# linusmossberg/monte-carlo-ray-tracer

Measured on NVIDIA H100. Metric: Mray/s (primary+shadow+bounce), higher is better.
Workload: dtype f64

## Files before the change

### include/mcrt_abi.h

```cpp
#ifndef MCRT_ABI_H
#define MCRT_ABI_H

#include <stddef.h>
#include <stdint.h>

#ifdef __cplusplus
extern "C" {
#endif

#define MCRT_ABI_VERSION 1

typedef enum mcrt_status {
    MCRT_OK = 0,
    MCRT_ERR_INVALID = -1,
    MCRT_ERR_CUDA = -2,
    MCRT_ERR_NO_SCENE = -3,
    MCRT_ERR_UNSUPPORTED = -4,
    MCRT_ERR_NO_PHOTONS = -5
} mcrt_status;

enum { MCRT_PRIM_TRIANGLE = 0, MCRT_PRIM_SPHERE = 1, MCRT_PRIM_QUADRIC = 2 };

enum { MCRT_INTEGRATOR_PATH = 0, MCRT_INTEGRATOR_PHOTON = 1 };

// ... 305 lines not shown
#define MCRT_DENOISE_DEFAULT_SIGMA_DEPTH 0.1
#define MCRT_DENOISE_DEFAULT_SIGMA_ALBEDO 0.1

int mcrt_denoise_dev(mcrt_ctx* ctx, const double* a_rgb_dev, const double* a_weight_dev,
                     const double* b_rgb_dev, const double* b_weight_dev, const uint32_t* tile_samples,
                     uint32_t tile, const double* features_dev, uint32_t width, uint32_t height,
                     const mcrt_denoise_params* params, double* out_rgb_dev, double* frame_error);

int mcrt_denoise_planes_dev(mcrt_ctx* ctx, const double* a_rgb_dev, const double* b_rgb_dev,
                            const double* a_planes_dev, const double* b_planes_dev, uint32_t n_planes,
                            const uint32_t* tile_samples, uint32_t tile, const double* features_dev,
                            uint32_t width, uint32_t height, const mcrt_denoise_params* params,
                            double* a_out_planes_dev, double* b_out_planes_dev,
                            double* out_rgb_dev, double* frame_error);

int mcrt_frame_alloc(mcrt_ctx* ctx, uint64_t bytes, void** dev_ptr, unsigned char ipc_handle[64]);
int mcrt_frame_open(mcrt_ctx* ctx, const unsigned char ipc_handle[64], void** dev_ptr);
int mcrt_frame_close(mcrt_ctx* ctx, void* peer_ptr);
int mcrt_frame_free(mcrt_ctx* ctx, void* dev_ptr);

int mcrt_bvh4_host(const mcrt_scene_desc* scene, uint32_t max_leaf, void** handle, const void** nodes128, uint32_t* n_nodes);
void mcrt_bvh4_host_free(void* handle);

int mcrt_fp64_peak(mcrt_ctx* ctx, double* dfma_per_second);

int mcrt_trace_closest(mcrt_ctx* ctx, const mcrt_ray* rays, size_t n, int precision,
                       mcrt_hit* hits, mcrt_stats* stats);

int mcrt_sample_rays(mcrt_ctx* ctx, const mcrt_ray* rays, const uint32_t* pixel,
                     const uint32_t* sample, size_t n, uint32_t global_seed,
                     int integrator_kind, int precision, double* out_rgb, mcrt_stats* stats);

int mcrt_sampler_stream(mcrt_ctx* ctx, const uint32_t* pixel, const uint32_t* sample, size_t n,
                        uint32_t n_shuffles, uint32_t global_seed, uint32_t* out_u32x7);

int mcrt_knn_search(mcrt_ctx* ctx, int which, const double* points_xyz, size_t n,
                    uint32_t* out_index, double* out_dist2, uint32_t* out_count,
                    mcrt_stats* stats);

int mcrt_set_option(mcrt_ctx* ctx, const char* key, double value);

#ifdef __cplusplus
}
#endif
#endif
```

### monte-carlo-ray-tracer_b200/__init__.py

```python
import ctypes as C
import math
import os
import struct

import numpy as np

HERE = os.path.dirname(os.path.abspath(__file__))
LIB_PATH = os.environ.get("MCRT_LIB", os.path.join(HERE, "libmcrt_b200.so"))

INTEGRATOR_PATH, INTEGRATOR_PHOTON = 0, 1
PRECISION_F64, PRECISION_F32 = 0, 1
PRIM_TRIANGLE, PRIM_SPHERE, PRIM_QUADRIC = 0, 1, 2
NO_PRIM = 0xFFFFFFFF

ABI_SYMBOLS = [
    "mcrt_abi_version", "mcrt_init", "mcrt_destroy", "mcrt_last_error", "mcrt_scene_upload",
    "mcrt_photon_upload", "mcrt_photon_emit", "mcrt_photon_download", "mcrt_octree_build",
    "mcrt_octree_free", "mcrt_render_rows", "mcrt_render_rows_dev", "mcrt_render_rows_strided_dev",
    "mcrt_trace_closest",
    "mcrt_sample_rays", "mcrt_sampler_stream", "mcrt_knn_search", "mcrt_set_option", "mcrt_set_film",
    "mcrt_obj_load", "mcrt_obj_free", "mcrt_obj_vertex_normals",
    "mcrt_bvh_build", "mcrt_bvh_free", "mcrt_image_tonemap", "mcrt_image_tonemap_dev",
    "mcrt_render_rows_strided_peers", "mcrt_frame_alloc", "mcrt_frame_open", "mcrt_frame_close", "mcrt_frame_free",
    "mcrt_render_film_sums_strided_dev", "mcrt_film_resolve_dev",
    "mcrt_bvh4_host", "mcrt_bvh4_host_free",
    "mcrt_fp64_peak", "mcrt_photon_emit_total", "mcrt_photon_emit_range", "mcrt_photon_build_dev",
    "mcrt_render_accumulate_dev", "mcrt_progressive_resolve_dev",
    "mcrt_render_accumulate_tiles_dev", "mcrt_progressive_resolve_tiles_dev",
    "mcrt_render_features_dev", "mcrt_denoise_dev", "mcrt_render_features_chain_dev",
    "mcrt_photon_emit_pass", "mcrt_photon_gather_radius", "mcrt_photon_gather_search",
    "mcrt_set_light_groups", "mcrt_render_accumulate_groups_dev", "mcrt_light_groups_combine_dev",
    "mcrt_render_accumulate_aovs_dev", "mcrt_photon_download_lights", "mcrt_render_accumulate_photon_components_dev",
    "mcrt_set_light_path_expressions", "mcrt_render_accumulate_lpe_dev", "mcrt_lpe_compile_host",
    "mcrt_lpe_compile_photon_host", "mcrt_photon_download_lpe_states", "mcrt_denoise_planes_dev",
]

AOV_NAMES = ("background", "emission", "diffuse_direct", "diffuse_indirect", "reflection_direct", "reflection_indirect",
             "transmission_direct", "transmission_indirect")

PHOTON_COMPONENT_NAMES = ("emission", "direct", "caustic", "global")

LPE_SYM_RD, LPE_SYM_RS, LPE_SYM_RG, LPE_SYM_TS, LPE_SYM_TG, LPE_SYM_B, LPE_SYM_L, LPE_SYM_LABEL0 = range(8)
LPE_DEAD, LPE_MAX_STATES, LPE_MAX_SYMBOLS, LPE_MAX_EXPRESSIONS = 255, 255, 71, 32
AOV_LPES = ("CB", "CL", "C<RD>[LB]", "C<RD>.+[LB]", "C[<RS><RG>][LB]", "C[<RS><RG>].+[LB]", "C<T.>[LB]", "C<T.>.+[LB]")


def PM_COMPONENT_LPES(direct_visualization):
    n = "[<RD><RG><TG>]"
# ... 161 lines not shown
        L.mcrt_photon_download.argtypes = [C.c_void_p, C.c_int, C.POINTER(PhotonMapDesc)]
        L.mcrt_photon_download_lights.argtypes = [C.c_void_p, C.c_int, C.c_void_p, C.c_uint64]
        L.mcrt_photon_download_lpe_states.argtypes = [C.c_void_p, C.c_int, C.c_void_p, C.c_uint64]
        L.mcrt_octree_build.argtypes = [C.c_void_p, C.c_void_p, C.c_uint64, C.c_uint32, C.c_void_p, C.POINTER(C.c_void_p),
                                        C.POINTER(PhotonMapDesc), C.POINTER(C.c_double)]
        L.mcrt_octree_free.argtypes = [C.c_void_p]
        L.mcrt_octree_free.restype = None
        render_args = [C.c_void_p, C.POINTER(CameraRec), C.c_uint32, C.c_uint32, C.c_uint32, C.c_uint32,
                       C.c_int, C.c_int, C.c_void_p, C.POINTER(Stats)]
        L.mcrt_render_rows.argtypes = render_args
        L.mcrt_render_rows_dev.argtypes = render_args
        L.mcrt_render_rows_strided_dev.argtypes = [C.c_void_p, C.POINTER(CameraRec), C.c_uint32, C.c_uint32, C.c_uint32,
                                                   C.c_uint32, C.c_uint32, C.c_int, C.c_int, C.c_void_p, C.POINTER(Stats)]
        L.mcrt_render_rows_strided_peers.argtypes = [C.c_void_p, C.POINTER(CameraRec), C.c_uint32, C.c_uint32, C.c_uint32, C.c_uint32,
                                                     C.c_uint32, C.c_int, C.c_int, C.c_void_p, C.c_uint32, C.c_int, C.POINTER(Stats)]
        L.mcrt_frame_alloc.argtypes = [C.c_void_p, C.c_uint64, C.POINTER(C.c_void_p), C.c_void_p]
        L.mcrt_frame_open.argtypes = [C.c_void_p, C.c_void_p, C.POINTER(C.c_void_p)]
        L.mcrt_frame_close.argtypes = [C.c_void_p, C.c_void_p]
        L.mcrt_frame_free.argtypes = [C.c_void_p, C.c_void_p]
        L.mcrt_fp64_peak.argtypes = [C.c_void_p, C.POINTER(C.c_double)]
        L.mcrt_bvh4_host.argtypes = [C.POINTER(SceneDesc), C.c_uint32, C.POINTER(C.c_void_p), C.POINTER(C.c_void_p), C.POINTER(C.c_uint32)]
        L.mcrt_bvh4_host_free.argtypes = [C.c_void_p]
        L.mcrt_bvh4_host_free.restype = None
        L.mcrt_render_film_sums_strided_dev.argtypes = [C.c_void_p, C.POINTER(CameraRec), C.c_uint32, C.c_uint32, C.c_uint32, C.c_uint32,
                                                        C.c_uint32, C.c_int, C.c_int, C.c_void_p, C.c_void_p, C.POINTER(Stats)]
        L.mcrt_film_resolve_dev.argtypes = [C.c_void_p, C.c_void_p, C.c_void_p, C.c_uint64, C.c_void_p]
        L.mcrt_render_accumulate_dev.argtypes = [C.c_void_p, C.POINTER(CameraRec), C.c_uint32, C.c_uint32, C.c_uint32, C.c_uint32,
                                                 C.c_uint32, C.c_uint32, C.c_int, C.c_int, C.c_void_p, C.c_void_p, C.POINTER(Stats)]
        L.mcrt_progressive_resolve_dev.argtypes = [C.c_void_p, C.c_void_p, C.c_void_p, C.c_uint64, C.c_void_p, C.c_void_p, C.c_uint64,
                                                   C.c_uint32, C.c_uint32, C.c_uint32, C.c_void_p, C.c_void_p, C.POINTER(C.c_double)]
        L.mcrt_render_accumulate_tiles_dev.argtypes = [C.c_void_p, C.POINTER(CameraRec), C.c_uint32, C.c_uint32, C.c_uint32, C.c_uint32,
                                                       C.c_void_p, C.c_uint32, C.c_uint32, C.c_uint32, C.c_int, C.c_int, C.c_void_p,
                                                       C.c_void_p, C.POINTER(Stats)]
        L.mcrt_progressive_resolve_tiles_dev.argtypes = [C.c_void_p, C.c_void_p, C.c_void_p, C.c_void_p, C.c_void_p, C.c_void_p,
                                                         C.c_uint32, C.c_uint32, C.c_uint32, C.c_void_p, C.c_void_p, C.c_void_p,
                                                         C.POINTER(C.c_double)]
        L.mcrt_set_light_groups.argtypes = [C.c_void_p, C.c_void_p, C.c_uint32, C.c_uint32]
        L.mcrt_render_accumulate_groups_dev.argtypes = [C.c_void_p, C.POINTER(CameraRec), C.c_uint32, C.c_uint32, C.c_uint32, C.c_uint32,
                                                        C.c_void_p, C.c_uint32, C.c_uint32, C.c_uint32, C.c_int, C.c_int, C.c_void_p,
                                                        C.c_uint32, C.POINTER(Stats)]
        L.mcrt_render_accumulate_aovs_dev.argtypes = L.mcrt_render_accumulate_groups_dev.argtypes
        L.mcrt_render_accumulate_photon_components_dev.argtypes = L.mcrt_render_accumulate_groups_dev.argtypes
        L.mcrt_set_light_path_expressions.argtypes = [C.c_void_p, C.c_void_p, C.c_uint32]
        L.mcrt_render_accumulate_lpe_dev.argtypes = L.mcrt_render_accumulate_groups_dev.argtypes
        L.mcrt_lpe_compile_host.argtypes = [C.c_void_p, C.c_uint32, C.c_uint32, C.c_void_p, C.c_void_p, C.c_void_p,
                                            C.POINTER(C.c_uint32), C.POINTER(C.c_uint32), C.c_char_p, C.c_uint32]
# ... 824 lines not shown
                   gpu_ms=ms.value, rounds=int(d.build_rounds), kernel_launches=int(d.kernel_launches))
        lib().mcrt_bvh_free(h)
        return out
    finally:
        lib().mcrt_destroy(ctx)


BVH4_NODE_DTYPE = np.dtype([("lo", "<f4", (3, 4)), ("hi", "<f4", (3, 4)), ("child", "<u4", (4,)), ("pad", "<u4", (4,))])


def bvh4_host(scene, max_leaf=0xFFFFFFFF):
    d = scene.desc()
    h, p, n = C.c_void_p(), C.c_void_p(), C.c_uint32()
    rc = lib().mcrt_bvh4_host(C.byref(d), max_leaf, C.byref(h), C.byref(p), C.byref(n))
    if rc:
        raise McrtError(f"mcrt_bvh4_host failed with {rc}")
    try:
        if n.value == 0:
            return np.zeros(0, BVH4_NODE_DTYPE)
        buf = (C.c_uint8 * (128 * n.value)).from_address(p.value)
        return np.frombuffer(buf, dtype=BVH4_NODE_DTYPE).copy()
    finally:
        lib().mcrt_bvh4_host_free(h)


def _lpe_strings(exprs):
    arr = (C.c_char_p * max(len(exprs), 1))()
    for i, e in enumerate(exprs):
        arr[i] = str(e).encode()
    return arr


def lpe_compile(exprs, n_groups=0):
    exprs = list(exprs)
    arr = _lpe_strings(exprs)
    nxt = np.zeros(LPE_MAX_STATES * LPE_MAX_SYMBOLS, np.uint8)
    acc = np.zeros(256, np.uint32)
    gs = np.zeros(max(int(n_groups), 1), np.uint8)
    ns, nsym = C.c_uint32(), C.c_uint32()
    err = C.create_string_buffer(1024)
    rc = lib().mcrt_lpe_compile_host(C.cast(arr, C.c_void_p) if exprs else None, len(exprs), int(n_groups),
                                     nxt.ctypes.data_as(C.c_void_p), acc.ctypes.data_as(C.c_void_p),
                                     gs.ctypes.data_as(C.c_void_p), C.byref(ns), C.byref(nsym), err, len(err))
    if rc:
        e = McrtError(f"mcrt_lpe_compile_host failed with {rc}: {err.value.decode()}")
        e.code = rc
# ... 596 lines not shown
```

### monte-carlo-ray-tracer_b200/csrc/abi.cu

```cuda
#include <algorithm>
#include <cmath>
#include <cstdio>
#include <cstdlib>
#include <cstring>
#include <string>
#include <vector>

#include "mcrt_abi.h"
#include "launch.h"
#include "bvh_build.h"
#include "image.h"
#include "denoise.h"
#include "lpe.h"

using namespace mcrt;

static const int MCRT_INTERNAL_EMIT = 100;

#define CK(call)                                                                              \
    do {                                                                                      \
        cudaError_t e_ = (call);                                                              \
        if (e_ != cudaSuccess)                                                                \
        {                                                                                     \
            ctx->error = std::string(#call) + ": " + cudaGetErrorString(e_);                  \
            return MCRT_ERR_CUDA;                                                             \
        }                                                                                     \
    } while (0)
// ... 16 lines not shown
    {
        PathBuffer<R> buf[2];
        ShadowRecord<R>* shadow = nullptr;
        V4<R>* hits = nullptr;
        uint32_t capacity = 0;
    };
}

struct mcrt_ctx
{
    int device = 0;
    int sm_count = 132;
    cudaStream_t stream = nullptr;
    std::string error;

    bool has_scene = false;
    std::vector<void*> scene_allocs;
    DeviceScene<double> scene64;
    DeviceScene<float> scene32;
    float scene_scale = 1.0f;
    uint32_t n_bvh4_nodes = 0;
    uint32_t bvh4_max_leaf = 0xFFFFFFFFu;
    int dynamic_fetch = -1;
    PeerFrames peer_out{};
    int exact_traversal = 0;

    WaveBuffers<double> wave64;
    WaveBuffers<float> wave32;
    std::vector<void*> wave_allocs64, wave_allocs32;

    uint32_t* d_sobol_bytes = nullptr;
    Counters* d_counters = nullptr;
    Counters* h_counters = nullptr;
    double* d_film = nullptr;
    size_t film_values = 0;
    bool film_default = true;
    mcrt_film film = {MCRT_FILM_BOX, 0u, 0.5};
    double* d_film_wsum = nullptr;
    size_t film_wsum_values = 0;
    double* d_film_cache = nullptr;
    double* d_host_out = nullptr;
    size_t host_out_values = 0;
    double* d_resolve_scratch = nullptr;
    size_t resolve_scratch_values = 0;
    double* d_denoise_scratch = nullptr;
    size_t denoise_scratch_values = 0;
// ... 392 lines not shown
                {
                    if (!leafRef(kids[c], n.child[c])) return 1;
                }
                else queue.push_back({ kids[c], self, (uint32_t)c });
            }
            out[self] = n;
            return 0;
        };
        std::vector<Item> kids;
        out.emplace_back();
        if (s.node_prim_count[0]) kids.push_back(itemOfNode(0));
        else childrenOf(0, kids);
        bool too_big = emit(kids, 0) != 0;
        for (size_t q = 0; q < queue.size() && !too_big; q++)
        {
            const Pending pn = queue[q];
            const uint32_t self = (uint32_t)out.size();
            out.emplace_back();
            out[pn.parent].child[pn.slot] = self;
            expand(pn.item, kids);
            too_big = emit(kids, self) != 0;
        }
        if (too_big) out.clear();
        return MCRT_OK;
    }

    template <class R>
    int uploadArrays(mcrt_ctx* ctx, const mcrt_scene_desc& s, SceneArrays<R>& a, uint64_t& bytes)
    {
        DeviceScene<R>& d = a.dev;
        int rc;
        if ((rc = devUpload(ctx, ctx->scene_allocs, &d.wide, a.wide, bytes))) return rc;
        if ((rc = devUpload(ctx, ctx->scene_allocs, &d.geom, a.geom, bytes))) return rc;
        if ((rc = devUpload(ctx, ctx->scene_allocs, &d.shade, a.shade, bytes))) return rc;
        if ((rc = devUpload(ctx, ctx->scene_allocs, &d.vnormals, a.vnormals, bytes))) return rc;
        if ((rc = devUpload(ctx, ctx->scene_allocs, &d.quadrics, a.quadrics, bytes))) return rc;
        if ((rc = devUpload(ctx, ctx->scene_allocs, &d.materials, a.materials, bytes))) return rc;
        if ((rc = devUpload(ctx, ctx->scene_allocs, &d.lights, a.lights, bytes))) return rc;
        {
            std::vector<uint32_t> combos;
            std::vector<uint8_t> cls(s.n_prims ? s.n_prims : 1, 1);
            for (uint32_t i = 0; i < s.n_prims; i++)
            {
                const uint32_t combo = (a.materials[a.shade[i].material].flags << 1) | (a.shade[i].vn_index >= 0 ? 1u : 0u);
                size_t k = 0;
                while (k < combos.size() && combos[k] != combo) k++;
// ... 526 lines not shown
            ctx->error = name + ": a reconstruction filter needs weight_sum_dev";
            return MCRT_ERR_INVALID;
        }
        return MCRT_OK;
    }
}

extern "C" int mcrt_photon_upload(mcrt_ctx* ctx, const mcrt_photon_map_desc* caustic_map, const mcrt_photon_map_desc* global_map,
                                  uint32_t k_nearest, uint32_t direct_visualization, uint64_t* h2d_bytes);

extern "C"
{

int mcrt_abi_version(void) { return MCRT_ABI_VERSION; }

int mcrt_init(int device, mcrt_ctx** out_ctx)
{
    if (!out_ctx) return MCRT_ERR_INVALID;
    *out_ctx = nullptr;
    int count = 0;
    if (cudaGetDeviceCount(&count) != cudaSuccess || device < 0 || device >= count) return MCRT_ERR_CUDA;
    mcrt_ctx* ctx = new mcrt_ctx();
    if (const char* e = std::getenv("MCRT_BVH4_MAX_LEAF")) ctx->bvh4_max_leaf = (uint32_t)std::atoi(e);
    ctx->device = device;
    auto fail = [&](int rc) { mcrt_destroy(ctx); return rc; };
    if (cudaSetDevice(device) != cudaSuccess) return fail(MCRT_ERR_CUDA);
    cudaDeviceProp prop;
    if (cudaGetDeviceProperties(&prop, device) != cudaSuccess) return fail(MCRT_ERR_CUDA);
    ctx->sm_count = prop.multiProcessorCount;
    if (cudaStreamCreateWithFlags(&ctx->stream, cudaStreamNonBlocking) != cudaSuccess) return fail(MCRT_ERR_CUDA);
    if (cudaMalloc((void**)&ctx->d_counters, sizeof(Counters)) != cudaSuccess) return fail(MCRT_ERR_CUDA);
    if (cudaMallocHost((void**)&ctx->h_counters, 2 * sizeof(Counters)) != cudaSuccess) return fail(MCRT_ERR_CUDA);
    {
        std::vector<uint32_t> tab(6 * 4 * 256);
        makeSobolByteTable(tab.data());
        if (cudaMalloc((void**)&ctx->d_sobol_bytes, tab.size() * 4) != cudaSuccess) return fail(MCRT_ERR_CUDA);
        if (cudaMemcpy(ctx->d_sobol_bytes, tab.data(), tab.size() * 4, cudaMemcpyHostToDevice) != cudaSuccess) return fail(MCRT_ERR_CUDA);
    }
    if (cudaEventCreate(&ctx->ev_start) != cudaSuccess || cudaEventCreate(&ctx->ev_stop) != cudaSuccess) return fail(MCRT_ERR_CUDA);
    for (int i = 0; i < 2; i++)
        if (cudaEventCreateWithFlags(&ctx->ev_poll[i], cudaEventDisableTiming) != cudaSuccess) return fail(MCRT_ERR_CUDA);
    *out_ctx = ctx;
    return MCRT_OK;
}

void mcrt_destroy(mcrt_ctx* ctx)
// ... 35 lines not shown
    delete ctx;
}

const char* mcrt_last_error(const mcrt_ctx* ctx)
{
    return ctx ? ctx->error.c_str() : "null context";
}

int mcrt_set_option(mcrt_ctx* ctx, const char* key, double value)
{
    if (!ctx || !key) return MCRT_ERR_INVALID;
    std::string k(key);
    if (k == "pool_paths") { if (value < 1024 || value > 268435456.0) return MCRT_ERR_INVALID; ctx->pool_paths = (uint32_t)value; }
    else if (k == "blocks_per_sm") { if (value < 1 || value > 32) return MCRT_ERR_INVALID; ctx->blocks_per_sm = (int)value; }
    else if (k == "ray_eps_scale") { if (value <= 0) return MCRT_ERR_INVALID; ctx->ray_eps_scale = value; }
    else if (k == "poll_interval") { if (value < 1 || value > 1024) return MCRT_ERR_INVALID; ctx->poll_interval = (int)value; }
    else if (k == "stage_timing") { ctx->stage_timing = value != 0.0; }
    else if (k == "sort_rays") { ctx->sort_rays = value != 0.0; }
    else if (k == "sort_shade") { ctx->sort_shade = value != 0.0; }
    else if (k == "sort_shade_class") { ctx->sort_shade_class = value != 0.0; }
    else if (k == "sort_prim_key") { ctx->sort_prim_key = (int)value; }
    else if (k == "exact_traversal") { ctx->exact_traversal = value != 0.0; }
    else if (k == "dynamic_fetch") { ctx->dynamic_fetch = (int)value; }
    else if (k == "bvh4_max_leaf") { if (value < 0 || value > 255) return MCRT_ERR_INVALID; ctx->bvh4_max_leaf = (uint32_t)value; }
    else { ctx->error = "unknown option " + k; return MCRT_ERR_INVALID; }
    return MCRT_OK;
}

int mcrt_scene_upload(mcrt_ctx* ctx, const mcrt_scene_desc* scene, uint64_t* h2d_bytes)
{
    if (!ctx) return MCRT_ERR_INVALID;
    if (!scene || scene->abi_version != MCRT_ABI_VERSION) { ctx->error = "scene description missing or ABI version mismatch"; return MCRT_ERR_INVALID; }
    if (scene->n_prims == 0 || scene->n_materials == 0) { ctx->error = "empty scene"; return MCRT_ERR_INVALID; }
    if (scene->n_prims >= (1u << 24)) { ctx->error = "more than 2^24 primitives"; return MCRT_ERR_UNSUPPORTED; }
    CK(cudaSetDevice(ctx->device));
    const mcrt_scene_desc& s = *scene;

    for (uint32_t i = 0; i < s.n_nodes; i++)
    {
        if (s.node_next_sibling[i] != 0 && (s.node_next_sibling[i] <= i || s.node_next_sibling[i] >= s.n_nodes))
        { ctx->error = "node_next_sibling must point forward"; return MCRT_ERR_INVALID; }
        if ((uint64_t)s.node_first_prim[i] + s.node_prim_count[i] > s.n_prims)
        { ctx->error = "node primitive range out of bounds"; return MCRT_ERR_INVALID; }
        if (s.node_prim_count[i] == 0 && i + 1 >= s.n_nodes)
        { ctx->error = "inner node without children"; return MCRT_ERR_INVALID; }
    }
// ... 34 lines not shown
                double a[3] = { sp[0] - sp[3], sp[1] - sp[3], sp[2] - sp[3] }, b[3] = { sp[0] + sp[3], sp[1] + sp[3], sp[2] + sp[3] };
                add(a); add(b);
            }
            for (uint32_t i = 0; i < s.n_quadrics; i++) { add(s.quadric_bounds + 6 * i); add(s.quadric_bounds + 6 * i + 3); }
        }
        for (int k = 0; k < 3; k++)
        {
            const bool ok = lo[k] <= hi[k] && lo[k] > -1e290 && hi[k] < 1e290;
            ctx->scene_bmin[k] = ok ? lo[k] : -1.0;
            ctx->scene_bmax[k] = ok ? hi[k] : 1.0;
        }
    }

    uint64_t bytes = 0;
    int rc;
    {
        SceneArrays<double> a;
        if ((rc = buildArrays(ctx, s, a))) return rc;
        std::memset(&a.dev, 0, sizeof(a.dev));
        if ((rc = buildWide(ctx, s, a))) return rc;
        if ((rc = uploadArrays(ctx, s, a, bytes))) return rc;
        std::vector<Bvh4Node> bvh4;
        if ((rc = buildBvh4(ctx->bvh4_max_leaf, s, bvh4))) return rc;
        a.dev.bvh4 = nullptr;
        if (!bvh4.empty() && (rc = devUpload(ctx, ctx->scene_allocs, &a.dev.bvh4, bvh4, bytes))) return rc;
        ctx->n_bvh4_nodes = (uint32_t)bvh4.size();
        CK(cudaStreamSynchronize(ctx->stream));
        ctx->scene64 = a.dev;
    }
    {
        SceneArrays<float> a;
        if ((rc = buildArrays(ctx, s, a))) return rc;
        std::memset(&a.dev, 0, sizeof(a.dev));
        if ((rc = buildWide(ctx, s, a))) return rc;
        if ((rc = uploadArrays(ctx, s, a, bytes))) return rc;
        CK(cudaStreamSynchronize(ctx->stream));
        ctx->scene32 = a.dev;
    }
    ctx->prim_interpolates.assign(s.n_prims, 0);
    for (uint32_t i = 0; i < s.n_prims; i++)
        if (s.prim_type[i] == MCRT_PRIM_TRIANGLE && s.tri_vn_index[s.prim_index[i]] >= 0) ctx->prim_interpolates[i] = 1;
    {
        std::vector<uint8_t> lit(s.n_prims, 0);
        for (uint32_t i = 0; i < s.n_lights; i++) lit[s.light_prim[i]] = 1;
        ctx->emissive_unlit = false;
        for (uint32_t i = 0; i < s.n_prims && !ctx->emissive_unlit; i++)
            ctx->emissive_unlit = s.materials[s.prim_material[i]].emissive && !lit[i];
    }
    ctx->has_scene = true;
// ... 1196 lines not shown
{
    if (!ctx) return MCRT_ERR_INVALID;
    if (!rgb_sum_dev || !weight_sum_dev || !out_rgb_dev) { ctx->error = "null buffer"; return MCRT_ERR_INVALID; }
    CK(cudaSetDevice(ctx->device));
    launchResolveFilmWeighted(rgb_sum_dev, weight_sum_dev, out_rgb_dev, n_pixels, ctx->sm_count * ctx->blocks_per_sm, ctx->stream);
    CK(cudaStreamSynchronize(ctx->stream));
    CK(cudaGetLastError());
    return MCRT_OK;
}

int mcrt_bvh4_host(const mcrt_scene_desc* scene, uint32_t max_leaf, void** handle, const void** nodes128, uint32_t* n_nodes)
{
    if (!scene || !handle || !nodes128 || !n_nodes) return MCRT_ERR_INVALID;
    auto* v = new std::vector<Bvh4Node>();
    const int rc = buildBvh4(max_leaf, *scene, *v);
    if (rc) { delete v; return rc; }
    *handle = v; *nodes128 = v->data(); *n_nodes = (uint32_t)v->size();
    return MCRT_OK;
}

void mcrt_bvh4_host_free(void* handle)
{
    delete static_cast<std::vector<Bvh4Node>*>(handle);
}

int mcrt_lpe_compile_host(const char* const* exprs, uint32_t n, uint32_t n_groups, uint8_t* next, uint32_t* accept,
                          uint8_t* group_symbol, uint32_t* n_states, uint32_t* n_symbols, char* error, uint32_t error_capacity)
{
    if (!next || !accept || !n_states || !n_symbols || (n_groups && !group_symbol)) return MCRT_ERR_INVALID;
    LpeTable t;
    std::string why;
    const int rc = lpeCompile(exprs, n, n_groups, t, why);
    if (error && error_capacity)
    {
        const size_t len = std::min<size_t>(why.size(), error_capacity - 1);
        std::memcpy(error, why.data(), len);
        error[len] = '\0';
    }
    if (rc != MCRT_OK) return rc;
    std::memcpy(next, t.next.data(), t.next.size());
    std::memcpy(accept, t.accept.data(), 256 * sizeof(uint32_t));
    for (uint32_t g = 0; g < n_groups; g++)
    {
        auto it = std::lower_bound(t.labels.begin(), t.labels.end(), g);
        group_symbol[g] = (uint8_t)(it != t.labels.end() && *it == g ? MCRT_LPE_SYM_LABEL0 + (it - t.labels.begin()) : MCRT_LPE_SYM_L);
    }
// ... 311 lines not shown
```

### monte-carlo-ray-tracer_b200/csrc/bvh4.cuh

```cuda
#pragma once

#include "intersect.cuh"

#ifndef MCRT_FAST_STACK
#define MCRT_FAST_STACK 40
#endif
#ifndef MCRT_SPECULATIVE
#define MCRT_SPECULATIVE 0
#endif
#ifndef MCRT_FAST_SMEM_STACK
#define MCRT_FAST_SMEM_STACK 0
#endif

namespace mcrt
{
    constexpr uint32_t BVH4_LEAF = 0x80000000u;
    constexpr uint32_t BVH4_MAX_PRIMS = 1u << 23;
    constexpr int FAST_STACK = MCRT_FAST_STACK;
    constexpr int FAST_SMEM_STACK = MCRT_FAST_SMEM_STACK;
    constexpr int FAST_LOCAL_STACK = FAST_STACK - FAST_SMEM_STACK;
    inline size_t fastStackSharedBytes(int block_threads) { return (size_t)FAST_SMEM_STACK * block_threads * sizeof(uint2); }

    struct alignas(16) Bvh4Node
    {
// ... 8 lines not shown
    {
        float idx, idy, idz;
        float onx, ony, onz;
        float ofx, ofy, ofz;
        uint32_t near_row[3];
    };

    MCRT_D FastRay makeFastRay(const V3<double>& o, const V3<double>& d)
    {
        FastRay r;
        auto inv = [](double v) { float f = (float)v; if (!(fabsf(f) >= 1e-18f)) f = copysignf(1e-18f, f); return 1.0f / f; };
        r.idx = inv(d.x); r.idy = inv(d.y); r.idz = inv(d.z);
        const float ox = (float)o.x * r.idx, oy = (float)o.y * r.idy, oz = (float)o.z * r.idz;
        const float mx = fabsf(ox) * 1.9073486e-6f, my = fabsf(oy) * 1.9073486e-6f, mz = fabsf(oz) * 1.9073486e-6f;
        r.onx = ox + mx; r.ony = oy + my; r.onz = oz + mz;
        r.ofx = ox - mx; r.ofy = oy - my; r.ofz = oz - mz;
        r.near_row[0] = r.idx < 0.0f ? 3u : 0u;
        r.near_row[1] = r.idy < 0.0f ? 3u : 0u;
        r.near_row[2] = r.idz < 0.0f ? 3u : 0u;
        return r;
    }

    template <int PRIMS, class R>
    MCRT_D bool intersectPrim(const DeviceScene<R>& sc, uint32_t prim, const RayQ<R>& ray, R& t, R& u, R& v, bool& is_triangle)
    {
        const V4<R> g0 = sc.geom[3 * prim + 0];
        const uint32_t type = PRIMS == PRIMS_TRI ? (uint32_t)PRIM_TRIANGLE : (uint32_t)g0.w;
        u = R(0); v = R(0);
        is_triangle = type == PRIM_TRIANGLE;
        if (type == PRIM_TRIANGLE)
        {
            const V4<R> g1 = sc.geom[3 * prim + 1];
            const V4<R> g2 = sc.geom[3 * prim + 2];
            return intersectTriangle(g0, g1, g2, ray, t, u, v);
        }
        else if (PRIMS == PRIMS_TRI_SPHERE || type == PRIM_SPHERE)
        {
            const V4<R> g1 = sc.geom[3 * prim + 1];
            return intersectSphere(g0, g1, ray, t);
        }
        else
        {
            return intersectQuadric(sc.quadrics[(uint32_t)g0.x], ray, t);
        }
    }

    MCRT_D double ambiguityDelta(double t, double scene_scale) { return 1e-6 * t + 1e-12 * scene_scale; }

    MCRT_D bool degenerateDirection(const V3<double>& d)
    {
        return fabs(d.x) < 1e-12 || fabs(d.y) < 1e-12 || fabs(d.z) < 1e-12;
    }
    MCRT_D bool onTriangleBoundary(double u, double v, double t, double scene_scale)
    {
        const double e = 1e-9 * fmax(1.0, t / scene_scale);
        return u < e || v < e || u + v > 1.0 - e;
    }

    template <int PRIMS, bool OCC = false> struct FastSearch
    {
        Hit<double> best;
        double second_t;
        float limit;
        int sp;
        uint32_t cur;
        FastRay fr;
        uint2 lstack[FAST_LOCAL_STACK > 0 ? FAST_LOCAL_STACK : 1];
        uint2* sstack;
        uint32_t target;
        uint32_t verdict;
        bool degenerate;

        MCRT_D bool beginOcclusion(const DeviceScene<double>& sc, const RayQ<double>& ray, uint32_t target_prim, TraceCounters& cnt)
        {
            best.u = 0.0; best.v = 0.0; best.interpolate = 0; best.prim = NO_PRIM; best.t = Consts<double>::MAXV;
            second_t = Consts<double>::MAXV;
            target = target_prim; verdict = 0u;
            sp = 0; cur = 0;
            attach();
            double t, u, v;
            bool is_tri;
            cnt.prim_tests++;
            if (!intersectPrim<PRIMS>(sc, target_prim, ray, t, u, v, is_tri)) return false;
            best.t = t; best.u = u; best.v = v; best.prim = target_prim;
            degenerate = degenerateDirection(ray.d) || (is_tri && onTriangleBoundary(u, v, t, (double)sc.scene_scale));
            if (degenerate) { verdict = 2u; return true; }
            limit = __double2float_ru(t + 2.0 * ambiguityDelta(t, (double)sc.scene_scale));
            fr = makeFastRay(ray.o, ray.d);
            return true;
        }

        MCRT_D void begin(const RayQ<double>& ray)
        {
            best.t = Consts<double>::MAXV; best.u = 0.0; best.v = 0.0; best.prim = NO_PRIM; best.interpolate = 0;
            second_t = Consts<double>::MAXV;
            limit = __int_as_float(0x7f800000);
            sp = 0;
            cur = 0;
            degenerate = degenerateDirection(ray.d);
            attach();
            fr = makeFastRay(ray.o, ray.d);
        }

        MCRT_D void attach()
        {
            extern __shared__ uint2 fast_stack_smem[];
// ... 45 lines not shown

            #define MCRT_CE(A, B) { const uint32_t lo_ = min(A, B); B = max(A, B); A = lo_; }
            MCRT_CE(key0, key1) MCRT_CE(key2, key3) MCRT_CE(key0, key2) MCRT_CE(key1, key3) MCRT_CE(key1, key2)
            #undef MCRT_CE
            auto refOf = [&](uint32_t key) { const uint32_t s = key & 3u; return s == 0u ? ch.x : (s == 1u ? ch.y : (s == 2u ? ch.z : ch.w)); };

            if (key0 == 0xFFFFFFFFu) return pop();
            if (key3 != 0xFFFFFFFFu) push(refOf(key3), key3 & ~3u);
            if (key2 != 0xFFFFFFFFu) push(refOf(key2), key2 & ~3u);
            if (key1 != 0xFFFFFFFFu) push(refOf(key1), key1 & ~3u);
            cur = refOf(key0);
            return true;
        }

        MCRT_D bool testLeaf(uint32_t leaf, const DeviceScene<double>& sc, const RayQ<double>& ray, TraceCounters& cnt)
        {
            const uint32_t first = (leaf >> 8) & (BVH4_MAX_PRIMS - 1u), count = leaf & 0xFFu;
            for (uint32_t i = first; i < first + count; i++)
            {
                double t, u, v;
                bool is_tri;
                if constexpr (OCC)
                {
                    if (i == target) continue;
                    if (intersectPrim<PRIMS>(sc, i, ray, t, u, v, is_tri))
                    {
                        const double delta = ambiguityDelta(best.t, (double)sc.scene_scale);
                        if (t <= best.t + delta && is_tri && onTriangleBoundary(u, v, t, (double)sc.scene_scale)) { verdict = 2u; cnt.prim_tests += i - first + 1; return false; }
                        if (t < best.t - delta) { verdict = 1u; cnt.prim_tests += i - first + 1; return false; }
                        if (t <= best.t + delta) { verdict = 2u; cnt.prim_tests += i - first + 1; return false; }
                    }
                    continue;
                }
                if (intersectPrim<PRIMS>(sc, i, ray, t, u, v, is_tri))
                {
                    if (t < best.t)
                    {
                        second_t = best.t;
                        best.t = t; best.u = u; best.v = v; best.prim = i;
                        best.interpolate = (is_tri && onTriangleBoundary(u, v, t, (double)sc.scene_scale)) ? 1u : 0u;
                        limit = __double2float_ru(t + 2.0 * ambiguityDelta(t, (double)sc.scene_scale));
                    }
                    else if (t < second_t)
                    {
                        second_t = t;
                    }
                }
            }
            cnt.prim_tests += count;
            return true;
        }

        MCRT_D bool step(const DeviceScene<double>& sc, const RayQ<double>& ray, TraceCounters& cnt)
        {
#if MCRT_SPECULATIVE
            uint32_t stashed = 0u;
            bool have_cur = true;
            while (true)
            {
                if (cur & BVH4_LEAF)
                {
                    if (stashed) break;
                    stashed = cur;
                    have_cur = pop();
                    if (!have_cur) break;
                }
// ... 124 lines not shown
```

### monte-carlo-ray-tracer_b200/csrc/scene.cuh

```cuda
#pragma once

#include "vec.cuh"

namespace mcrt
{
    constexpr uint32_t NO_PRIM = 0xFFFFFFFFu;
    constexpr uint32_t WIDE_LEAF = 0x80000000u;

    enum PrimType : uint32_t { PRIM_TRIANGLE = 0, PRIM_SPHERE = 1, PRIM_QUADRIC = 2 };

    template <class R> struct WideChild;
    template <> struct alignas(16) WideChild<float>
    {
        float bmin[3];
        float bmax[3];
        uint32_t a, b;
    };
    template <> struct alignas(16) WideChild<double>
    {
        double bmin[3];
        double bmax[3];
        uint32_t a, b;
        uint32_t _pad[2];
    };
// ... 26 lines not shown

    enum MaterialFlags : uint32_t
    {
        MAT_COMPLEX_IOR = 1u, MAT_PERFECT_MIRROR = 2u, MAT_ROUGH = 4u, MAT_ROUGH_SPECULAR = 8u,
        MAT_OPAQUE = 16u, MAT_EMISSIVE = 32u, MAT_DIRAC_DELTA = 64u
    };

    template <class R> struct alignas(16) Light
    {
        V3<R> p0, p1, p2;
        V3<R> normal;
        V3<R> emittance;
        R area;
        R cdf;
        uint32_t prim;
        uint32_t type;
    };

    struct Bvh4Node;

    template <class R> struct DeviceScene
    {
        const Bvh4Node* bvh4;
        const WideChild<R>* wide;
        const V4<R>* geom;
        const PrimShade<R>* shade;
        const V4<R>* vnormals;
        const Quadric<R>* quadrics;
        const Material<R>* materials;
        const Light<R>* lights;
        const uint8_t* shade_class;
        uint32_t n_nodes, n_prims, n_lights, n_wide_root;
        uint32_t root_is_leaf, root_first_prim, root_prim_count;
        uint32_t prims_class;
        uint32_t dynamic_fetch;
        uint32_t _pad3[2];
        uint32_t material_flags_any;
        R root_bmin[3], root_bmax[3];
        R scene_ior;
        R scene_scale;
    };

    template <class R> struct DeviceCamera
    {
        V3<R> eye, forward, left, up;
        R focal_length, sensor_width, aperture_radius, focus_distance;
// ... 11 lines not shown
```

Measured before the change: 2837.

## Build spatial-split SBVH for BVH4 with duplicated primitive references

Adds a host-side SBVH builder that considers spatial splits, clipping triangles against bin planes, alongside binned SAH object splits, under a reference budget. The result is collapsed into the BVH4 layout together with a reference-to-primitive index array and a reordered per-reference geometry buffer. It is enabled by default for small scenes (under 4096 primitives, default max-leaf setting). Traversal now reads geometry through the ref buffer and maps refs back to primitive ids. The aim is tighter node bounds and fewer wasted box and primitive tests, at the cost of duplicated references, an extra index load per hit or occlusion check, and a longer build.

```diff
diff --git a/include/mcrt_abi.h b/include/mcrt_abi.h
--- a/include/mcrt_abi.h
+++ b/include/mcrt_abi.h
@@ -351,6 +351,10 @@
 int mcrt_bvh4_host(const mcrt_scene_desc* scene, uint32_t max_leaf, void** handle, const void** nodes128, uint32_t* n_nodes);
 void mcrt_bvh4_host_free(void* handle);
 
+int mcrt_bvh4_split_host(const mcrt_scene_desc* scene, double node_cost, double ref_budget, void** handle, const void** nodes128,
+                         uint32_t* n_nodes, const uint32_t** refs, uint32_t* n_refs);
+void mcrt_bvh4_split_host_free(void* handle);
+
 int mcrt_fp64_peak(mcrt_ctx* ctx, double* dfma_per_second);
 
 int mcrt_trace_closest(mcrt_ctx* ctx, const mcrt_ray* rays, size_t n, int precision,
diff --git a/monte-carlo-ray-tracer_b200/__init__.py b/monte-carlo-ray-tracer_b200/__init__.py
--- a/monte-carlo-ray-tracer_b200/__init__.py
+++ b/monte-carlo-ray-tracer_b200/__init__.py
@@ -23,7 +23,7 @@
     "mcrt_bvh_build", "mcrt_bvh_free", "mcrt_image_tonemap", "mcrt_image_tonemap_dev",
     "mcrt_render_rows_strided_peers", "mcrt_frame_alloc", "mcrt_frame_open", "mcrt_frame_close", "mcrt_frame_free",
     "mcrt_render_film_sums_strided_dev", "mcrt_film_resolve_dev",
-    "mcrt_bvh4_host", "mcrt_bvh4_host_free",
+    "mcrt_bvh4_host", "mcrt_bvh4_host_free", "mcrt_bvh4_split_host", "mcrt_bvh4_split_host_free",
     "mcrt_fp64_peak", "mcrt_photon_emit_total", "mcrt_photon_emit_range", "mcrt_photon_build_dev",
     "mcrt_render_accumulate_dev", "mcrt_progressive_resolve_dev",
     "mcrt_render_accumulate_tiles_dev", "mcrt_progressive_resolve_tiles_dev",
@@ -231,6 +231,10 @@
         L.mcrt_bvh4_host.argtypes = [C.POINTER(SceneDesc), C.c_uint32, C.POINTER(C.c_void_p), C.POINTER(C.c_void_p), C.POINTER(C.c_uint32)]
         L.mcrt_bvh4_host_free.argtypes = [C.c_void_p]
         L.mcrt_bvh4_host_free.restype = None
+        L.mcrt_bvh4_split_host.argtypes = [C.POINTER(SceneDesc), C.c_double, C.c_double, C.POINTER(C.c_void_p), C.POINTER(C.c_void_p),
+                                           C.POINTER(C.c_uint32), C.POINTER(C.c_void_p), C.POINTER(C.c_uint32)]
+        L.mcrt_bvh4_split_host_free.argtypes = [C.c_void_p]
+        L.mcrt_bvh4_split_host_free.restype = None
         L.mcrt_render_film_sums_strided_dev.argtypes = [C.c_void_p, C.POINTER(CameraRec), C.c_uint32, C.c_uint32, C.c_uint32, C.c_uint32,
                                                         C.c_uint32, C.c_int, C.c_int, C.c_void_p, C.c_void_p, C.POINTER(Stats)]
         L.mcrt_film_resolve_dev.argtypes = [C.c_void_p, C.c_void_p, C.c_void_p, C.c_uint64, C.c_void_p]
@@ -1101,6 +1105,26 @@
         return np.frombuffer(buf, dtype=BVH4_NODE_DTYPE).copy()
     finally:
         lib().mcrt_bvh4_host_free(h)
+
+
+BVH4_SPLIT_NODE_COST = 0.5
+BVH4_SPLIT_REF_BUDGET = 2.0
+
+
+def bvh4_split_host(scene, node_cost=BVH4_SPLIT_NODE_COST, ref_budget=BVH4_SPLIT_REF_BUDGET):
+    d = scene.desc()
+    h, p, n, r, nr = C.c_void_p(), C.c_void_p(), C.c_uint32(), C.c_void_p(), C.c_uint32()
+    rc = lib().mcrt_bvh4_split_host(C.byref(d), float(node_cost), float(ref_budget), C.byref(h), C.byref(p), C.byref(n), C.byref(r), C.byref(nr))
+    if rc:
+        raise McrtError(f"mcrt_bvh4_split_host failed with {rc}")
+    try:
+        if n.value == 0:
+            return np.zeros(0, BVH4_NODE_DTYPE), np.zeros(0, np.uint32)
+        nodes = np.frombuffer((C.c_uint8 * (128 * n.value)).from_address(p.value), dtype=BVH4_NODE_DTYPE).copy()
+        refs = np.frombuffer((C.c_uint8 * (4 * nr.value)).from_address(r.value), dtype=np.uint32).copy()
+        return nodes, refs
+    finally:
+        lib().mcrt_bvh4_split_host_free(h)
 
 
 def _lpe_strings(exprs):
diff --git a/monte-carlo-ray-tracer_b200/csrc/abi.cu b/monte-carlo-ray-tracer_b200/csrc/abi.cu
--- a/monte-carlo-ray-tracer_b200/csrc/abi.cu
+++ b/monte-carlo-ray-tracer_b200/csrc/abi.cu
@@ -3,6 +3,7 @@
 #include <cstdio>
 #include <cstdlib>
 #include <cstring>
+#include <functional>
 #include <string>
 #include <vector>
 
@@ -65,6 +66,8 @@
     uint32_t n_bvh4_nodes = 0;
     uint32_t bvh4_max_leaf = 0xFFFFFFFFu;
     int dynamic_fetch = -1;
+    int bvh4_split = -1;
+    double bvh4_split_cost = 0.5;
     PeerFrames peer_out{};
     int exact_traversal = 0;
 
@@ -503,6 +506,271 @@
             too_big = emit(kids, self) != 0;
         }
         if (too_big) out.clear();
+        return MCRT_OK;
+    }
+
+    int buildBvh4Split(const mcrt_scene_desc& s, double node_cost, double ref_budget, std::vector<Bvh4Node>& out, std::vector<uint32_t>& refs)
+    {
+        out.clear(); refs.clear();
+        if (s.n_nodes == 0 || s.n_prims == 0 || s.n_prims >= BVH4_MAX_PRIMS) return MCRT_OK;
+        auto lower = [](double v) { float r = (float)v; if ((double)r > v) r = std::nextafter(r, -INFINITY); return r; };
+        auto upper = [](double v) { float r = (float)v; if ((double)r < v) r = std::nextafter(r, INFINITY); return r; };
+        struct Ref { uint32_t prim; double b[6]; };
+        struct SNode { double b[6]; int32_t kid[2]; uint32_t first, count; };
+        constexpr int NB = 32;
+        constexpr uint32_t MAX_LEAF = 2;
+        const double eps = std::ldexp(1.0, -40);
+        auto empty = [](double* b) { for (int k = 0; k < 3; k++) { b[k] = 1e300; b[3 + k] = -1e300; } };
+        auto grow = [](double* b, const double* c) { for (int k = 0; k < 3; k++) { b[k] = std::min(b[k], c[k]); b[3 + k] = std::max(b[3 + k], c[3 + k]); } };
+        auto area = [](const double* b) { const double x = b[3] - b[0], y = b[4] - b[1], z = b[5] - b[2]; return (x < 0 || y < 0 || z < 0) ? 0.0 : x * y + y * z + z * x; };
+        auto isEmpty = [](const double* b) { return b[0] > b[3] || b[1] > b[4] || b[2] > b[5]; };
+        auto vert = [&](const double* base, uint32_t idx, double* p) { for (int k = 0; k < 3; k++) p[k] = base[3 * (size_t)idx + k]; };
+
+        auto clip = [&](uint32_t prim, const double* c, double* out_b)
+        {
+            empty(out_b);
+            const uint32_t type = s.prim_type[prim], idx = s.prim_index[prim];
+            if (type == MCRT_PRIM_TRIANGLE)
+            {
+                struct P { double x[3]; double e; };
+                P poly[16], next[16];
+                int n = 3;
+                vert(s.tri_v0, idx, poly[0].x); vert(s.tri_v1, idx, poly[1].x); vert(s.tri_v2, idx, poly[2].x);
+                for (int i = 0; i < 3; i++) poly[i].e = 0.0;
+                for (int plane = 0; plane < 6 && n > 0; plane++)
+                {
+                    const int k = plane % 3;
+                    const bool is_lo = plane < 3;
+                    const double pos = c[plane];
+                    auto inside = [&](const P& p) { return is_lo ? p.x[k] >= pos : p.x[k] <= pos; };
+                    int m = 0;
+                    for (int i = 0; i < n; i++)
+                    {
+                        const P& a = poly[i];
+                        const P& b = poly[(i + 1) % n];
+                        const bool ia = inside(a), ib = inside(b);
+                        if (ia) next[m++] = a;
+                        if (ia != ib)
+                        {
+                            const double den = b.x[k] - a.x[k];
+                            const double t = std::min(1.0, std::max(0.0, (pos - a.x[k]) / den));
+                            P q;
+                            double span = 0.0;
+                            for (int j = 0; j < 3; j++) { q.x[j] = a.x[j] + t * (b.x[j] - a.x[j]); span = std::max(span, std::fabs(b.x[j] - a.x[j])); }
+                            q.x[k] = pos;
+                            const double mag = std::fabs(pos) + std::fabs(a.x[k]) + std::fabs(b.x[k]);
+                            q.e = std::max(a.e, b.e) + span * std::min(1.0, eps * mag / std::fabs(den)) +
+                                  eps * (std::fabs(q.x[0]) + std::fabs(q.x[1]) + std::fabs(q.x[2]) + span);
+                            next[m++] = q;
+                        }
+                    }
+                    n = m;
+                    for (int i = 0; i < n; i++) poly[i] = next[i];
+                }
+                for (int i = 0; i < n; i++)
+                    for (int k = 0; k < 3; k++)
+                    {
+                        out_b[k] = std::min(out_b[k], poly[i].x[k] - poly[i].e - eps * std::fabs(poly[i].x[k]));
+                        out_b[3 + k] = std::max(out_b[3 + k], poly[i].x[k] + poly[i].e + eps * std::fabs(poly[i].x[k]));
+                    }
+            }
+            else
+            {
+                const double* sp = s.sphere_origin_radius + 4 * (size_t)idx;
+                for (int k = 0; k < 3; k++) { out_b[k] = sp[k] - sp[3]; out_b[3 + k] = sp[k] + sp[3]; }
+            }
+            for (int k = 0; k < 3; k++) { out_b[k] = std::max(out_b[k], c[k]); out_b[3 + k] = std::min(out_b[3 + k], c[3 + k]); }
+        };
+        auto cut = [&](const Ref& r, int k, double pos, Ref& l, Ref& rr)
+        {
+            double c[6];
+            l.prim = rr.prim = r.prim;
+            std::memcpy(c, r.b, sizeof(c)); c[3 + k] = std::min(c[3 + k], pos); clip(r.prim, c, l.b);
+            std::memcpy(c, r.b, sizeof(c)); c[k] = std::max(c[k], pos); clip(r.prim, c, rr.b);
+        };
+
+        std::vector<Ref> all(s.n_prims);
+        bool quadrics = false;
+        for (uint32_t i = 0; i < s.n_prims; i++)
+        {
+            Ref& r = all[i];
+            r.prim = i;
+            const uint32_t type = s.prim_type[i], idx = s.prim_index[i];
+            if (type == MCRT_PRIM_TRIANGLE)
+            {
+                double v[3][3];
+                vert(s.tri_v0, idx, v[0]); vert(s.tri_v1, idx, v[1]); vert(s.tri_v2, idx, v[2]);
+                for (int k = 0; k < 3; k++) { r.b[k] = std::min(v[0][k], std::min(v[1][k], v[2][k])); r.b[3 + k] = std::max(v[0][k], std::max(v[1][k], v[2][k])); }
+            }
+            else if (type == MCRT_PRIM_SPHERE)
+            {
+                const double* sp = s.sphere_origin_radius + 4 * (size_t)idx;
+                for (int k = 0; k < 3; k++) { r.b[k] = sp[k] - sp[3]; r.b[3 + k] = sp[k] + sp[3]; }
+            }
+            else { quadrics = true; for (int k = 0; k < 6; k++) r.b[k] = s.quadric_bounds[6 * (size_t)idx + k]; }
+        }
+        const size_t budget = (size_t)(ref_budget * s.n_prims);
+        size_t n_refs = all.size();
+        std::vector<SNode> nodes;
+
+        std::function<int32_t(std::vector<Ref>&)> build = [&](std::vector<Ref>& rs) -> int32_t
+        {
+            SNode nd;
+            empty(nd.b);
+            for (const Ref& r : rs) grow(nd.b, r.b);
+            nd.kid[0] = nd.kid[1] = -1; nd.first = 0; nd.count = (uint32_t)rs.size();
+            const int32_t self = (int32_t)nodes.size();
+            nodes.push_back(nd);
+            const size_t n = rs.size();
+            auto makeLeaf = [&]() { nodes[self].first = (uint32_t)refs.size(); for (const Ref& r : rs) refs.push_back(r.prim); return self; };
+            if (n <= 1) return makeLeaf();
+            const double pa = std::max(area(nd.b), 1e-300);
+            double best = INFINITY; int best_axis = -1, best_bin = -1; bool best_spatial = false;
+            double cbox[6]; empty(cbox);
+            for (const Ref& r : rs) for (int k = 0; k < 3; k++) { const double cc = 0.5 * (r.b[k] + r.b[3 + k]); cbox[k] = std::min(cbox[k], cc); cbox[3 + k] = std::max(cbox[3 + k], cc); }
+            auto centroidBin = [&](const Ref& r, int k) { const double ext = cbox[3 + k] - cbox[k]; int b = (int)(NB * ((0.5 * (r.b[k] + r.b[3 + k]) - cbox[k]) / ext)); return std::min(NB - 1, std::max(0, b)); };
+            for (int k = 0; k < 3; k++)
+            {
+                if (!(cbox[3 + k] > cbox[k])) continue;
+                double bb[NB][6]; uint32_t cnt[NB] = {};
+                for (int b = 0; b < NB; b++) empty(bb[b]);
+                for (const Ref& r : rs) { const int b = centroidBin(r, k); grow(bb[b], r.b); cnt[b]++; }
+                double right[NB][6]; uint32_t rc[NB];
+                double acc[6]; empty(acc); uint32_t ac = 0;
+                for (int b = NB - 1; b >= 1; b--) { grow(acc, bb[b]); ac += cnt[b]; std::memcpy(right[b], acc, sizeof(acc)); rc[b] = ac; }
+                empty(acc); ac = 0;
+                for (int b = 0; b < NB - 1; b++)
+                {
+                    grow(acc, bb[b]); ac += cnt[b];
+                    if (ac == 0 || rc[b + 1] == 0) continue;
+                    const double cost = node_cost + (area(acc) * ac + area(right[b + 1]) * rc[b + 1]) / pa;
+                    if (cost < best) { best = cost; best_axis = k; best_bin = b; best_spatial = false; }
+                }
+            }
+            bool has_quadric = false;
+            if (quadrics) for (const Ref& r : rs) has_quadric |= s.prim_type[r.prim] == MCRT_PRIM_QUADRIC;
+            if (!has_quadric && n_refs + n <= budget)
+            {
+                for (int k = 0; k < 3; k++)
+                {
+                    const double lo = nd.b[k], ext = nd.b[3 + k] - nd.b[k];
+                    if (!(ext > 0.0)) continue;
+                    auto plane = [&](int b) { return lo + ext * b / NB; };
+                    auto binOf = [&](double x) { return std::min(NB - 1, std::max(0, (int)(NB * ((x - lo) / ext)))); };
+                    double bb[NB][6]; uint32_t enter[NB] = {}, leave[NB] = {};
+                    for (int b = 0; b < NB; b++) empty(bb[b]);
+                    for (const Ref& r : rs)
+                    {
+                        const int b0 = binOf(r.b[k]), b1 = binOf(r.b[3 + k]);
+                        enter[b0]++; leave[b1]++;
+                        Ref cur = r, l, rr;
+                        for (int b = b0; b < b1; b++)
+                        {
+                            cut(cur, k, plane(b + 1), l, rr);
+                            if (!isEmpty(l.b)) grow(bb[b], l.b);
+                            cur = rr;
+                            if (isEmpty(cur.b)) break;
+                        }
+                        if (!isEmpty(cur.b)) grow(bb[b1], cur.b);
+                    }
+                    double right[NB][6]; uint32_t rc[NB];
+                    double acc[6]; empty(acc); uint32_t ac = 0;
+                    for (int b = NB - 1; b >= 1; b--) { grow(acc, bb[b]); ac += leave[b]; std::memcpy(right[b], acc, sizeof(acc)); rc[b] = ac; }
+                    empty(acc); ac = 0;
+                    for (int b = 0; b < NB - 1; b++)
+                    {
+                        grow(acc, bb[b]); ac += enter[b];
+                        if (ac == 0 || rc[b + 1] == 0 || (ac == n && rc[b + 1] == n)) continue;
+                        const double cost = node_cost + (area(acc) * ac + area(right[b + 1]) * rc[b + 1]) / pa;
+                        if (cost < best) { best = cost; best_axis = k; best_bin = b; best_spatial = true; }
+                    }
+                }
+            }
+            if (n <= MAX_LEAF && (double)n <= best) return makeLeaf();
+            std::vector<Ref> ls, rrs;
+            if (best_spatial)
+            {
+                const int k = best_axis;
+                const double lo = nd.b[k], ext = nd.b[3 + k] - nd.b[k];
+                const double pos = lo + ext * (best_bin + 1) / NB;
+                for (const Ref& r : rs)
+                {
+                    if (r.b[3 + k] <= pos) ls.push_back(r);
+                    else if (r.b[k] >= pos) rrs.push_back(r);
+                    else
+                    {
+                        Ref l, rr;
+                        cut(r, k, pos, l, rr);
+                        if (!isEmpty(l.b)) ls.push_back(l);
+                        if (!isEmpty(rr.b)) rrs.push_back(rr);
+                    }
+                }
+                if (ls.empty() || rrs.empty() || (ls.size() == n && rrs.size() == n)) { ls.clear(); rrs.clear(); }
+                else n_refs += ls.size() + rrs.size() - n;
+            }
+            else if (best_axis >= 0)
+            {
+                for (const Ref& r : rs) (centroidBin(r, best_axis) <= best_bin ? ls : rrs).push_back(r);
+            }
+            if (ls.empty() || rrs.empty())
+            {
+                ls.clear(); rrs.clear();
+                int k = 0;
+                for (int j = 1; j < 3; j++) if (nd.b[3 + j] - nd.b[j] > nd.b[3 + k] - nd.b[k]) k = j;
+                std::vector<Ref> sorted = rs;
+                std::stable_sort(sorted.begin(), sorted.end(), [&](const Ref& a, const Ref& b) { return a.b[k] + a.b[3 + k] < b.b[k] + b.b[3 + k]; });
+                ls.assign(sorted.begin(), sorted.begin() + n / 2);
+                rrs.assign(sorted.begin() + n / 2, sorted.end());
+            }
+            rs.clear(); rs.shrink_to_fit();
+            const int32_t l = build(ls);
+            const int32_t r = build(rrs);
+            nodes[self].kid[0] = l; nodes[self].kid[1] = r;
+            return self;
+        };
+        build(all);
+        if (refs.size() >= BVH4_MAX_PRIMS) { out.clear(); refs.clear(); return MCRT_OK; }
+
+        auto isInner = [&](int32_t i) { return nodes[i].kid[0] >= 0; };
+        struct Pending { int32_t node; uint32_t parent, slot; };
+        std::vector<Pending> queue;
+        auto emit = [&](int32_t bnode, uint32_t self)
+        {
+            std::vector<int32_t> kids;
+            if (isInner(bnode)) kids = { nodes[bnode].kid[0], nodes[bnode].kid[1] };
+            else kids = { bnode };
+            while (kids.size() < 4)
+            {
+                int pick = -1; double pick_area = -1.0;
+                for (size_t i = 0; i < kids.size(); i++)
+                    if (isInner(kids[i]) && area(nodes[kids[i]].b) > pick_area) { pick_area = area(nodes[kids[i]].b); pick = (int)i; }
+                if (pick < 0) break;
+                const int32_t c = kids[pick];
+                kids[pick] = nodes[c].kid[0];
+                kids.insert(kids.begin() + pick + 1, nodes[c].kid[1]);
+            }
+            Bvh4Node n;
+            std::memset(&n, 0, sizeof(n));
+            for (int c = 0; c < 4; c++) for (int k = 0; k < 3; k++) { n.lo[k][c] = 3.0e38f; n.hi[k][c] = -3.0e38f; }
+            for (size_t c = 0; c < kids.size(); c++)
+            {
+                const SNode& sn = nodes[kids[c]];
+                for (int k = 0; k < 3; k++) { n.lo[k][c] = lower(sn.b[k]); n.hi[k][c] = upper(sn.b[3 + k]); }
+                if (!isInner(kids[c])) n.child[c] = BVH4_LEAF | (sn.first << 8) | sn.count;
+                else queue.push_back({ kids[c], self, (uint32_t)c });
+            }
+            out[self] = n;
+        };
+        out.emplace_back();
+        emit(0, 0);
+        for (size_t q = 0; q < queue.size(); q++)
+        {
+            const Pending pn = queue[q];
+            const uint32_t self = (uint32_t)out.size();
+            out.emplace_back();
+            out[pn.parent].child[pn.slot] = self;
+            emit(pn.node, self);
+        }
         return MCRT_OK;
     }
 
@@ -1075,6 +1343,8 @@
     if (cudaGetDeviceCount(&count) != cudaSuccess || device < 0 || device >= count) return MCRT_ERR_CUDA;
     mcrt_ctx* ctx = new mcrt_ctx();
     if (const char* e = std::getenv("MCRT_BVH4_MAX_LEAF")) ctx->bvh4_max_leaf = (uint32_t)std::atoi(e);
+    if (const char* e = std::getenv("MCRT_BVH4_SPLIT")) ctx->bvh4_split = std::atoi(e);
+    if (const char* e = std::getenv("MCRT_BVH4_SPLIT_COST")) ctx->bvh4_split_cost = std::atof(e);
     ctx->device = device;
     auto fail = [&](int rc) { mcrt_destroy(ctx); return rc; };
     if (cudaSetDevice(device) != cudaSuccess) return fail(MCRT_ERR_CUDA);
@@ -1156,6 +1426,7 @@
     else if (k == "sort_prim_key") { ctx->sort_prim_key = (int)value; }
     else if (k == "exact_traversal") { ctx->exact_traversal = value != 0.0; }
     else if (k == "dynamic_fetch") { ctx->dynamic_fetch = (int)value; }
+    else if (k == "bvh4_split") { if (value < -1 || value > 1) return MCRT_ERR_INVALID; ctx->bvh4_split = (int)value; }
     else if (k == "bvh4_max_leaf") { if (value < 0 || value > 255) return MCRT_ERR_INVALID; ctx->bvh4_max_leaf = (uint32_t)value; }
     else { ctx->error = "unknown option " + k; return MCRT_ERR_INVALID; }
     return MCRT_OK;
@@ -1236,9 +1507,35 @@
         if ((rc = uploadArrays(ctx, s, a, bytes))) return rc;
         std::vector<Bvh4Node> bvh4;
         if ((rc = buildBvh4(ctx->bvh4_max_leaf, s, bvh4))) return rc;
-        a.dev.bvh4 = nullptr;
-        if (!bvh4.empty() && (rc = devUpload(ctx, ctx->scene_allocs, &a.dev.bvh4, bvh4, bytes))) return rc;
         ctx->n_bvh4_nodes = (uint32_t)bvh4.size();
+        a.dev.bvh4 = nullptr; a.dev.bvh4_geom = nullptr; a.dev.bvh4_prim = nullptr;
+        std::vector<uint32_t> refs;
+        std::vector<V4<double>> ref_geom;
+        if (!bvh4.empty())
+        {
+            const bool split = ctx->bvh4_split < 0 ? ctx->bvh4_max_leaf == 0xFFFFFFFFu && s.n_prims < 4096u : ctx->bvh4_split != 0;
+            if (split)
+            {
+                std::vector<Bvh4Node> split_nodes;
+                if ((rc = buildBvh4Split(s, ctx->bvh4_split_cost, 2.0, split_nodes, refs))) return rc;
+                if (!split_nodes.empty()) bvh4.swap(split_nodes);
+                else refs.clear();
+            }
+            if (refs.empty())
+            {
+                refs.resize(s.n_prims);
+                for (uint32_t i = 0; i < s.n_prims; i++) refs[i] = i;
+                a.dev.bvh4_geom = a.dev.geom;
+            }
+            else
+            {
+                ref_geom.resize(3 * refs.size());
+                for (size_t r = 0; r < refs.size(); r++) for (int j = 0; j < 3; j++) ref_geom[3 * r + j] = a.geom[3 * (size_t)refs[r] + j];
+                if ((rc = devUpload(ctx, ctx->scene_allocs, &a.dev.bvh4_geom, ref_geom, bytes))) return rc;
+            }
+            if ((rc = devUpload(ctx, ctx->scene_allocs, &a.dev.bvh4_prim, refs, bytes))) return rc;
+            if ((rc = devUpload(ctx, ctx->scene_allocs, &a.dev.bvh4, bvh4, bytes))) return rc;
+        }
         CK(cudaStreamSynchronize(ctx->stream));
         ctx->scene64 = a.dev;
     }
@@ -2481,6 +2778,27 @@
 void mcrt_bvh4_host_free(void* handle)
 {
     delete static_cast<std::vector<Bvh4Node>*>(handle);
+}
+
+namespace
+{
+    struct Bvh4SplitHost { std::vector<Bvh4Node> nodes; std::vector<uint32_t> refs; };
+}
+
+int mcrt_bvh4_split_host(const mcrt_scene_desc* scene, double node_cost, double ref_budget, void** handle, const void** nodes128,
+                         uint32_t* n_nodes, const uint32_t** refs, uint32_t* n_refs)
+{
+    if (!scene || !handle || !nodes128 || !n_nodes || !refs || !n_refs || !(node_cost >= 0.0) || !(ref_budget >= 1.0)) return MCRT_ERR_INVALID;
+    auto* v = new Bvh4SplitHost();
+    const int rc = buildBvh4Split(*scene, node_cost, ref_budget, v->nodes, v->refs);
+    if (rc) { delete v; return rc; }
+    *handle = v; *nodes128 = v->nodes.data(); *n_nodes = (uint32_t)v->nodes.size(); *refs = v->refs.data(); *n_refs = (uint32_t)v->refs.size();
+    return MCRT_OK;
+}
+
+void mcrt_bvh4_split_host_free(void* handle)
+{
+    delete static_cast<Bvh4SplitHost*>(handle);
 }
 
 int mcrt_lpe_compile_host(const char* const* exprs, uint32_t n, uint32_t n_groups, uint8_t* next, uint32_t* accept,
diff --git a/monte-carlo-ray-tracer_b200/csrc/bvh4.cuh b/monte-carlo-ray-tracer_b200/csrc/bvh4.cuh
--- a/monte-carlo-ray-tracer_b200/csrc/bvh4.cuh
+++ b/monte-carlo-ray-tracer_b200/csrc/bvh4.cuh
@@ -54,21 +54,21 @@
     }
 
     template <int PRIMS, class R>
-    MCRT_D bool intersectPrim(const DeviceScene<R>& sc, uint32_t prim, const RayQ<R>& ray, R& t, R& u, R& v, bool& is_triangle)
-    {
-        const V4<R> g0 = sc.geom[3 * prim + 0];
+    MCRT_D bool intersectPrim(const DeviceScene<R>& sc, const V4<R>* __restrict__ geom, uint32_t prim, const RayQ<R>& ray, R& t, R& u, R& v, bool& is_triangle)
+    {
+        const V4<R> g0 = geom[3 * prim + 0];
         const uint32_t type = PRIMS == PRIMS_TRI ? (uint32_t)PRIM_TRIANGLE : (uint32_t)g0.w;
         u = R(0); v = R(0);
         is_triangle = type == PRIM_TRIANGLE;
         if (type == PRIM_TRIANGLE)
         {
-            const V4<R> g1 = sc.geom[3 * prim + 1];
-            const V4<R> g2 = sc.geom[3 * prim + 2];
+            const V4<R> g1 = geom[3 * prim + 1];
+            const V4<R> g2 = geom[3 * prim + 2];
             return intersectTriangle(g0, g1, g2, ray, t, u, v);
         }
         else if (PRIMS == PRIMS_TRI_SPHERE || type == PRIM_SPHERE)
         {
-            const V4<R> g1 = sc.geom[3 * prim + 1];
+            const V4<R> g1 = geom[3 * prim + 1];
             return intersectSphere(g0, g1, ray, t);
         }
         else
@@ -113,7 +113,7 @@
             double t, u, v;
             bool is_tri;
             cnt.prim_tests++;
-            if (!intersectPrim<PRIMS>(sc, target_prim, ray, t, u, v, is_tri)) return false;
+            if (!intersectPrim<PRIMS>(sc, sc.geom, target_prim, ray, t, u, v, is_tri)) return false;
             best.t = t; best.u = u; best.v = v; best.prim = target_prim;
             degenerate = degenerateDirection(ray.d) || (is_tri && onTriangleBoundary(u, v, t, (double)sc.scene_scale));
             if (degenerate) { verdict = 2u; return true; }
@@ -205,8 +205,8 @@
                 bool is_tri;
                 if constexpr (OCC)
                 {
-                    if (i == target) continue;
-                    if (intersectPrim<PRIMS>(sc, i, ray, t, u, v, is_tri))
+                    if (__ldg(sc.bvh4_prim + i) == target) continue;
+                    if (intersectPrim<PRIMS>(sc, sc.bvh4_geom, i, ray, t, u, v, is_tri))
                     {
                         const double delta = ambiguityDelta(best.t, (double)sc.scene_scale);
                         if (t <= best.t + delta && is_tri && onTriangleBoundary(u, v, t, (double)sc.scene_scale)) { verdict = 2u; cnt.prim_tests += i - first + 1; return false; }
@@ -215,16 +215,16 @@
                     }
                     continue;
                 }
-                if (intersectPrim<PRIMS>(sc, i, ray, t, u, v, is_tri))
+                if (intersectPrim<PRIMS>(sc, sc.bvh4_geom, i, ray, t, u, v, is_tri))
                 {
                     if (t < best.t)
                     {
                         second_t = best.t;
-                        best.t = t; best.u = u; best.v = v; best.prim = i;
+                        best.t = t; best.u = u; best.v = v; best.prim = __ldg(sc.bvh4_prim + i);
                         best.interpolate = (is_tri && onTriangleBoundary(u, v, t, (double)sc.scene_scale)) ? 1u : 0u;
                         limit = __double2float_ru(t + 2.0 * ambiguityDelta(t, (double)sc.scene_scale));
                     }
-                    else if (t < second_t)
+                    else if (t < second_t && !(t == best.t && __ldg(sc.bvh4_prim + i) == best.prim))
                     {
                         second_t = t;
                     }
diff --git a/monte-carlo-ray-tracer_b200/csrc/scene.cuh b/monte-carlo-ray-tracer_b200/csrc/scene.cuh
--- a/monte-carlo-ray-tracer_b200/csrc/scene.cuh
+++ b/monte-carlo-ray-tracer_b200/csrc/scene.cuh
@@ -72,6 +72,8 @@
     template <class R> struct DeviceScene
     {
         const Bvh4Node* bvh4;
+        const V4<R>* bvh4_geom;
+        const uint32_t* bvh4_prim;
         const WideChild<R>* wide;
         const V4<R>* geom;
         const PrimShade<R>* shade;
```

After: 2931, median of 6. +3.3%, better.
